# burn-research/OpenMEASURE

Hardware: AMD Instinct MI355X
Metric: SPR fit+reconstruct throughput (GB/s snapshot matrix) (higher is better)
Workload: dtype f64

## Files before the change

### include/spr_hip.h

```cpp
#ifndef SPR_HIP_H
#define SPR_HIP_H

#include <stddef.h>
#include <stdint.h>

#ifdef __cplusplus
extern "C" {
#endif

#define SPR_OK 0
#define SPR_E_INVALID (-1)
#define SPR_E_UNSUPPORTED (-2)
#define SPR_E_HIP (-3)
#define SPR_E_WORKSPACE (-4)

#define SPR_MAX_M 256
#define SPR_MAX_M_WIDE 512
#define SPR_MAX_R 128
#define SPR_MAX_R_STREAM 256
#define SPR_MAX_R_WIDE 1024

#define SPR_ABI_VERSION 5
int spr_abi_version(void);
const char *spr_last_error(void);
int spr_device_cus(int *out_cus);
int spr_upload_bytes(void *d_dst, const void *h_pinned_src, int64_t n_bytes, void *stream);
int spr_download_bytes(void *h_pinned_dst, const void *d_src, int64_t n_bytes, void *h_pinned_ticket, uint64_t ticket_value,
                       void *stream);
int spr_host_tridiag_vectors(const double *h_d, const double *h_e, int32_t m, const double *h_lam, int32_t r, double *h_Z,
                             int32_t iterations);
int spr_host_eig_top(const double *h_G, int32_t m, int32_t r, double *h_lam, double *h_V, void *fn_dsytrd, void *fn_dsterf,
                     void *fn_dormtr);
int spr_host_svd_top(const double *h_M, int32_t m, int32_t r, double *h_S, double *h_V, void *fn_dgebrd, void *fn_dbdsdc,
                     void *fn_dormbr);

size_t spr_stats_gram_workspace(int32_t m, int32_t n_features);
int spr_stats_gram_f64(const double *d_X, int64_t n_rows, int32_t m, int64_t ldx,
                       int64_t row0, int64_t n_points, int32_t n_features, int32_t center,
                       double *d_rowmean, void *d_workspace, size_t workspace_bytes, void *stream);
int spr_stats_gram_finalize_f64(int64_t n_rows, int32_t m, int64_t row0, int64_t n_points,
                                int32_t n_features, const void *d_workspace, size_t workspace_bytes,
                                double *d_fstats, double *d_gram, int32_t ldg, int32_t origin,
                                void *stream);
size_t spr_rowstats_workspace(int32_t n_features);
int spr_rowstats_f64(const double *d_X, int64_t n_rows, int32_t m, int64_t ldx, int64_t row0,
                     int64_t n_points, int32_t n_features, double *d_rowmean, double *d_fstats,
                     void *d_workspace, size_t workspace_bytes, void *stream);
size_t spr_gram_cross_workspace(int32_t m, int32_t n_features);
int spr_gram_cross_f64(const double *d_X, int64_t n_rows, int32_t m, int64_t ldx, int64_t row0,
                       int64_t n_points, int32_t n_features, int32_t center, double *d_rowmean,
                       double *d_gram, void *d_workspace, size_t workspace_bytes, void *stream);
int spr_rowmean_stats_f64(const double *d_rowmean, int64_t n_rows, int64_t row0, int64_t n_points,
                          int32_t n_features, double *d_fstats, void *d_workspace, size_t workspace_bytes,
                          void *stream);
int spr_gram_cross_pair_f64(const double *d_X, int64_t n_rows, int32_t col_a, int32_t col_b, int32_t w_b,
                            int32_t ldg, int64_t ldx, int64_t row0, int64_t n_points, int32_t n_features,
                            int32_t center, double *d_rowmean, double *d_gram, void *d_workspace,
                            size_t workspace_bytes, void *stream);

int32_t spr_spectrum_max_m(void);
int spr_spectrum_f64(const double *d_gram, const double *d_fstats_all, int32_t n_ranks,
                     int32_t n_features, int32_t m, int32_t scale_code, int32_t r, double *d_feat,
                     double *d_scale, double *d_inv_scale, double *d_lam, double *d_S, double *d_expvar,
                     double *d_V, double *d_W, double *d_Ar, double *d_info, void *stream);

int spr_gram_combine_f64(const double *d_gram, const double *d_fstats_all, int32_t n_ranks,
// ... 403 lines not shown
```

### openmeasure_amd/_lib.py

```python
from __future__ import annotations

import ctypes as C
import os

_HERE = os.path.dirname(os.path.abspath(__file__))
LIB_PATH = os.environ.get('SPR_HIP_LIBRARY') or os.path.join(_HERE, 'libspr_hip.so')

SPR_ABI_VERSION = 5
SPR_MAX_M = 256
SPR_MAX_M_WIDE = 512
SPR_MAX_R = 128
SPR_MAX_R_STREAM = 256
SPR_MAX_R_WIDE = 1024
SPR_GP_MAX_M = 800
SPR_GP_MAX_D = 8

_i32, _i64, _u64, _sz = C.c_int32, C.c_int64, C.c_uint64, C.c_size_t
_p = C.c_void_p
_dbl = C.c_double

PROTOTYPES = {
    'spr_abi_version': (C.c_int, []),
    'spr_last_error': (C.c_char_p, []),
    'spr_device_cus': (C.c_int, [C.POINTER(C.c_int)]),
    'spr_upload_bytes': (C.c_int, [_p, _p, _i64, _p]),
    'spr_download_bytes': (C.c_int, [_p, _p, _i64, _p, _u64, _p]),
    'spr_host_tridiag_vectors': (C.c_int, [_p, _p, _i32, _p, _i32, _p, _i32]),
    'spr_host_eig_top': (C.c_int, [_p, _i32, _i32, _p, _p, _p, _p, _p]),
    'spr_host_svd_top': (C.c_int, [_p, _i32, _i32, _p, _p, _p, _p, _p]),
    'spr_stats_gram_workspace': (_sz, [_i32, _i32]),
    'spr_stats_gram_f64': (C.c_int, [_p, _i64, _i32, _i64, _i64, _i64, _i32, _i32, _p, _p, _sz, _p]),
    'spr_stats_gram_finalize_f64': (C.c_int, [_i64, _i32, _i64, _i64, _i32, _p, _sz, _p, _p, _i32, _i32, _p]),
    'spr_stats_gram_shifted_f64': (C.c_int, [_p, _i64, _i32, _i64, _i64, _i64, _i32, _p, _p, _p, _sz, _p]),
    'spr_gram_shift_finish_f64': (C.c_int, [_p, _p, _i64, _i32, _i32, _p, _i32, _p]),
    'spr_rowstats_workspace': (_sz, [_i32]),
    'spr_rowstats_f64': (C.c_int, [_p, _i64, _i32, _i64, _i64, _i64, _i32, _p, _p, _p, _sz, _p]),
    'spr_gram_cross_workspace': (_sz, [_i32, _i32]),
    'spr_gram_cross_f64': (C.c_int, [_p, _i64, _i32, _i64, _i64, _i64, _i32, _i32, _p, _p, _p, _sz, _p]),
    'spr_gram_cross_pair_f64': (C.c_int, [_p, _i64, _i32, _i32, _i32, _i32, _i64, _i64, _i64, _i32, _i32, _p, _p, _p, _sz, _p]),
    'spr_rowmean_stats_f64': (C.c_int, [_p, _i64, _i64, _i64, _i32, _p, _p, _sz, _p]),
    'spr_spectrum_max_m': (_i32, []),
    'spr_spectrum_f64': (C.c_int, [_p, _p, _i32, _i32, _i32, _i32, _i32, _p, _p, _p, _p, _p, _p, _p, _p, _p, _p, _p]),
    'spr_gram_combine_f64': (C.c_int, [_p, _p, _i32, _i32, _i32, _i32, _p, _p, _p, _p, _p]),
    'spr_project_f64': (C.c_int, [_p, _i64, _i32, _i64, _i64, _i64, _i32, _i32, _p, _p, _p, _i32, _p, _i64, _i32, _p]),
    'spr_project_norms_supported': (_i32, [_i32, _i32, _i64, _i64, _p, _i32]),
    'spr_project_norms_f64': (C.c_int, [_p, _i64, _i32, _i64, _i64, _i64, _i32, _i32, _p, _p, _p, _i32, _p, _i64, _p, _p]),
    'spr_project_stream_norms_f64': (C.c_int, [_p, _i64, _i32, _i64, _i64, _i64, _i32, _i32, _p, _p, _p, _i32, _p, _i64, _p, _p, _sz, _p]),
    'spr_project_stream_workspace': (_sz, [_i32, _i32, _i32]),
    'spr_project_stream_f64': (C.c_int, [_p, _i64, _i32, _i64, _i64, _i64, _i32, _i32, _p, _p, _p, _i32, _p, _i64, _p, _sz, _p]),
    'spr_scale_rows_f64': (C.c_int, [_p, _i64, _i32, _i64, _i64, _i64, _i32, _p, _p, _p, _i64, _p]),
    'spr_unscale_f64': (C.c_int, [_p, _i64, _i64, _i64, _i32, _p, _p, _p, _p, _p]),
    'spr_feature_minmax_workspace': (_sz, [_i32]),
    'spr_feature_minmax_f64': (C.c_int, [_p, _i64, _i32, _i64, _i64, _i64, _i32, _p, _p, _sz, _p]),
    'spr_feature_digit_hist_f64': (C.c_int, [_p, _i64, _i32, _i64, _i64, _i64, _i32, _p, _i32, _i32, _i32, _p, _p]),
    'spr_colsums_workspace': (_sz, [_i32, _i32]),
# ... 152 lines not shown
```

### openmeasure_amd/csrc/project_ws.hip

```cpp
#include <type_traits>

#include "rowtile.hpp"
#include "launch.hpp"

namespace {

#ifndef WS_ABLATE
#define WS_ABLATE 0
#endif
constexpr int WS_WAVES = 8;
constexpr int WS_ROWS = 16 * WS_WAVES;

template <int RT> struct WsLds { static constexpr int NC = 16 * RT, LDW = NC; static_assert(RT % 2 == 0, "column tiles come in pairs"); };

template <typename TX> struct WsPiece;
template <> struct WsPiece<double> { f64x2 a, b; };
template <> struct WsPiece<float> { float x, y, z, w; };

template <int VEC, typename TX>
__device__ inline WsPiece<TX> ws_load(const TX *__restrict__ rp, int col0, int m) {
  WsPiece<TX> p;
  if constexpr (std::is_same<TX, double>::value) {
    if (VEC) {
      p.a = *reinterpret_cast<const f64x2 *>(rp + col0);
      p.b = *reinterpret_cast<const f64x2 *>(rp + col0 + 2);
    } else {
      p.a.x = rp[col0 < m ? col0 : 0];         p.a.y = rp[col0 + 1 < m ? col0 + 1 : 0];
      p.b.x = rp[col0 + 2 < m ? col0 + 2 : 0]; p.b.y = rp[col0 + 3 < m ? col0 + 3 : 0];
    }
  } else {
    if (VEC) {
      const float4 v = *reinterpret_cast<const float4 *>(rp + col0);
      p.x = v.x; p.y = v.y; p.z = v.z; p.w = v.w;
    } else {
      p.x = rp[col0 < m ? col0 : 0];         p.y = rp[col0 + 1 < m ? col0 + 1 : 0];
      p.z = rp[col0 + 2 < m ? col0 + 2 : 0]; p.w = rp[col0 + 3 < m ? col0 + 3 : 0];
    }
  }
  return p;
}

template <typename TX>
__device__ inline double ws_elem(const WsPiece<TX> &p, int t) {
  if constexpr (std::is_same<TX, double>::value) return t == 0 ? p.a.x : t == 1 ? p.a.y : t == 2 ? p.b.x : p.b.y;
  else return (double)(t == 0 ? p.x : t == 1 ? p.y : t == 2 ? p.z : p.w);
}

template <int MT, int RT, int VEC, typename TX, typename TU, bool NRM>
__global__ __launch_bounds__(WS_WAVES * 64) void project_ws_kernel(
    const TX *__restrict__ X, int64_t ldx, int m, int center_i, SegPlan plan, const double *__restrict__ inv_scale,
    const double *__restrict__ rowmean, const double *__restrict__ W, int r, TU *__restrict__ Ur, int64_t ldu,
    double *__restrict__ nrm2) {
  constexpr int K = 16 * MT, NJ = MT;
  constexpr int NC = WsLds<RT>::NC, LDW = WsLds<RT>::LDW;
  __shared__ double Wl[K * LDW];

  int f, wl, wpf, base;
  int64_t lo, hi;
  if (!seg_locate(plan, blockIdx.x, f, wl, wpf, base, lo, hi)) return;

  const int lane = threadIdx.x & 63;
  const int wave = __builtin_amdgcn_readfirstlane(threadIdx.x >> 6);
  const int li = lane & 15, kk = lane >> 4;
  const double isc = inv_scale[f];

  for (int e = threadIdx.x; e < K * NC; e += WS_WAVES * 64) {
    const int k = e / NC, c = e - k * NC;
    Wl[k * LDW + (c >> 5) * 32 + (c & 15) * 2 + ((c >> 4) & 1)] = (k < m && c < r) ? W[(int64_t)k * r + c] * isc : 0.0;
  }
  __syncthreads();
  double wbar[RT];
#pragma unroll
  for (int ct = 0; ct < RT; ++ct) {
    double sacc = 0.0;
    if (center_i != 0) {
      for (int k = kk; k < K; k += 4) sacc += Wl[k * LDW + (ct >> 1) * 32 + li * 2 + (ct & 1)];
      sacc += __shfl_xor(sacc, 16, 64);
      sacc += __shfl_xor(sacc, 32, 64);
    }
    wbar[ct] = sacc;
  }

  const int64_t nchunks = (hi - lo + WS_ROWS - 1) / WS_ROWS;
  int64_t c = wl;
  if (c >= nchunks) return;
  const double *wb = Wl + (4 * kk) * LDW + 2 * li;
  const double *wb_hi = wb + 128 * LDW;

  auto row_ptr = [&](int64_t cc) {
    int64_t row = lo + cc * WS_ROWS + 16 * wave + li;
    row = row < hi ? row : hi - 1;
    return X + row * ldx;
  };
  WsPiece<TX> areg[NJ];
  {
    const TX *rp = row_ptr(c);
#pragma unroll
    for (int j = 0; j < NJ; ++j) areg[j] = ws_load<VEC, TX>(rp, 16 * j + 4 * kk, m);
  }
  while (c < nchunks) {
    const int64_t cn = c + wpf;
    const TX *rpn = row_ptr(cn < nchunks ? cn : c);
    const int64_t blk0 = lo + c * WS_ROWS + 16 * wave;
    double mu[4];
#pragma unroll
    for (int i = 0; i < 4; ++i) {
      const int64_t rr = blk0 + kk + 4 * i;
      const double v = rowmean[rr < hi ? rr : hi - 1];
// ... 43 lines not shown
        if (NRM) {
#pragma unroll
          for (int i = 0; i < 4; ++i) { const double v = (double)(TU)s[i]; q[i] = fma(v, v, q[i]); }
        }
        if (full) {
#pragma unroll
          for (int i = 0; i < 4; ++i) up[4 * i * ldu + 16 * ct] = (TU)s[i];
        } else if (16 * ct + li < r) {
#pragma unroll
          for (int i = 0; i < 4; ++i)
            if (blk0 + kk + 4 * i < hi) up[4 * i * ldu + 16 * ct] = (TU)s[i];
        }
      }
      if (NRM) {
#pragma unroll
        for (int i = 0; i < 4; ++i) {
          const double t = group_sum_t<16>(q[i]);
          if (li == i && blk0 + kk + 4 * i < hi) nrm2[blk0 + kk + 4 * i] = t;
        }
      }
    }
    c = cn;
  }
}

template <int MT, int RT, typename TX, typename TU>
int ws_launch(const TX *X, int64_t n_rows, int32_t m, int64_t ldx, int64_t row0, int64_t n_points, int32_t n_features,
              int center, const double *inv_scale, const double *rowmean, const double *W, int32_t r, TU *Ur,
              int64_t ldu, int accumulate, double *nrm2, hipStream_t st) {
  SegPlan plan = spr_make_plan(row0, n_rows, n_points, n_features, WS_ROWS);
  static const int narrow_per_cu = [] { const char *e = getenv("SPR_WS_WG_PER_CU"); const int v = e ? atoi(e) : 2; return v >= 1 && v <= 4 ? v : 2; }();
  const int grid = spr_plan_grid(plan, MT <= 4 ? narrow_per_cu : 1);
  const bool vec = (m == 16 * MT) && spr_rows_aligned16(X, sizeof(TX) * ldx);
  if (!vec) return SPR_E_UNSUPPORTED;
  if (nrm2)
    hipLaunchKernelGGL((project_ws_kernel<MT, RT, 1, TX, TU, true>), dim3(grid), dim3(WS_WAVES * 64), 0, st, X, ldx, (int)m,
                       center, plan, inv_scale, rowmean, W, (int)r, Ur, ldu, nrm2);
  else
    hipLaunchKernelGGL((project_ws_kernel<MT, RT, 1, TX, TU, false>), dim3(grid), dim3(WS_WAVES * 64), 0, st, X, ldx, (int)m,
                       center, plan, inv_scale, rowmean, W, (int)r, Ur, ldu, nrm2);
  SPR_LAUNCH_CHECK();
  return SPR_OK;
}

}

#include "project_ws.hpp"

template <typename TX, typename TU>
int spr_project_ws(const TX *d_X, int64_t n_rows, int32_t m, int64_t ldx, int64_t row0, int64_t n_points,
                   int32_t n_features, int32_t center, const double *d_inv_scale, const double *d_rowmean,
                   const double *d_W, int32_t r, TU *d_Ur, int64_t ldu, int32_t accumulate, double *d_rownorm2,
                   hipStream_t st) {
  if (accumulate) return SPR_E_UNSUPPORTED;
  const int mt = spr_round_mt(m);
  const int need = (r + 15) / 16;
  const int rt = need <= 2 ? 2 : need <= 4 ? 4 : 0;
#define WS(MTV, RTV)                                                                                             \
  if (mt == MTV && rt == RTV)                                                                                    \
    return ws_launch<MTV, RTV, TX, TU>(d_X, n_rows, m, ldx, row0, n_points, n_features, center, d_inv_scale,   \
                                        d_rowmean, d_W, r, d_Ur, ldu, accumulate, d_rownorm2, st)
#ifdef PROJ_WS_LAB
  WS(16, 4);
// ... 19 lines not shown
```

### openmeasure_amd/csrc/stats_gram.hip

```cpp
#include <stdlib.h>

#include <type_traits>

#include "rowtile.hpp"
#include "launch.hpp"

#ifndef GRAM_UNIT_PAIRING
#define GRAM_UNIT_PAIRING 1
#endif
#ifndef GRAM_ABLATE
#define GRAM_ABLATE 0
#endif
#if GRAM_ABLATE == 1
#define GRAM_MFMA(a, b, c) ({ asm volatile("" ::"v"(a), "v"(b)); (c); })
#else
#define GRAM_MFMA(a, b, c) __builtin_amdgcn_mfma_f64_16x16x4f64((a), (b), (c), 0, 0, 0)
#endif

namespace {

template <int MT>
struct GramShape {
  static constexpr int MPAD = 16 * MT;
  static constexpr int MP = MPAD + ((MT % 2 == 0) ? 16 : 0);
  static constexpr int T = MT * (MT + 1) / 2;
  static constexpr int NU = (MT + 1) / 2;
};

// ... 11 lines not shown
template <> struct GramCfg<12> { static constexpr int NW = 12, R = 24, KS = 2; static constexpr bool DBUF = false; static constexpr int LPRMAX = 32; };
#ifndef GRAM_DBUF16
#define GRAM_DBUF16 false
#endif
template <> struct GramCfg<16> { static constexpr int NW = 8,  R = 32, KS = 1; static constexpr bool DBUF = GRAM_DBUF16; static constexpr int LPRMAX = 16; };

template <int MT> struct GramOut { static constexpr int KSO = (GramCfg<MT>::KS >= 4) ? 1 : GramCfg<MT>::KS; };

constexpr int tri_index(int mt, int ti, int tj) { return ti * mt - ti * (ti - 1) / 2 + (tj - ti); }

template <int MT>
__device__ inline void tile_coords(int idx, int &ti, int &tj) {
  ti = 0;
  while (ti < MT - 1 && idx >= MT - ti) { idx -= MT - ti; ++ti; }
  tj = ti + idx;
  if (tj > MT - 1) tj = MT - 1;
}

template <int MT, int U, int VEC, typename TX>
__device__ inline void gram_wave(const TX *__restrict__ X, int64_t ldx, int m, int center,
                                 int64_t lo, int64_t hi, int wl, int wpf, int ks, int wave, int lane,
                                 double *__restrict__ lds0, double *__restrict__ lds1,
                                 double *__restrict__ rowmean, double *__restrict__ stat_part,
                                 double *__restrict__ slab, double *__restrict__ rowsum) {
  using S = GramShape<MT>;
  using C = GramCfg<MT>;
  constexpr int R = C::R, KS = C::KS, NW = C::NW, MP = S::MP, T = S::T;
  constexpr int KROWS = R / KS, KSTEPS = KROWS / 4;
  constexpr int RA = U, RB = MT - 1 - U;
  constexpr int NA = MT - RA;
  constexpr int NB = (RB != RA) ? MT - RB : 0;
  static_assert(KROWS % 4 == 0, "k slice must be a multiple of the MFMA depth");
  using RT = RowTile<MT, R, MP, NW, C::LPRMAX, TX>;

  f64x4 accA[NA];
  f64x4 accB[NB > 0 ? NB : 1];
#pragma unroll
  for (int j = 0; j < NA; ++j) accA[j] = (f64x4){0.0, 0.0, 0.0, 0.0};
#pragma unroll
  for (int j = 0; j < NB; ++j) accB[j] = (f64x4){0.0, 0.0, 0.0, 0.0};

  RowStats st;
  st.init();
  RT tile;

  const int64_t nchunks = (hi - lo + R - 1) / R;
  int64_t c = wl;
// ... 77 lines not shown
        }
#pragma unroll
        for (int j = 0; j < NB; ++j) {
          double *tp = red + tri_index(MT, RB, RB + j) * 256;
          tp[0] = accB[j].x; tp[64] = accB[j].y; tp[128] = accB[j].z; tp[192] = accB[j].w;
        }
      }
      __syncthreads();
      if (ks == s - 1) {
#pragma unroll
        for (int j = 0; j < NA; ++j) {
          const double *tp = red + tri_index(MT, RA, RA + j) * 256;
          accA[j].x += tp[0]; accA[j].y += tp[64]; accA[j].z += tp[128]; accA[j].w += tp[192];
        }
#pragma unroll
        for (int j = 0; j < NB; ++j) {
          const double *tp = red + tri_index(MT, RB, RB + j) * 256;
          accB[j].x += tp[0]; accB[j].y += tp[64]; accB[j].z += tp[128]; accB[j].w += tp[192];
        }
      }
    }
  }
  if (KSO == KS || ks == 0) {
    double *sp = slab + ((int64_t)blockIdx.x * KSO + (KSO == KS ? ks : 0)) * T * 256 + lane;
#pragma unroll
    for (int j = 0; j < NA; ++j) {
      double *tp = sp + (int64_t)tri_index(MT, RA, RA + j) * 256;
      tp[0] = accA[j].x; tp[64] = accA[j].y; tp[128] = accA[j].z; tp[192] = accA[j].w;
    }
#pragma unroll
    for (int j = 0; j < NB; ++j) {
      double *tp = sp + (int64_t)tri_index(MT, RB, RB + j) * 256;
      tp[0] = accB[j].x; tp[64] = accB[j].y; tp[128] = accB[j].z; tp[192] = accB[j].w;
    }
  }
  if ((lane % RT::LPR) == 0) {
    double *q = stat_part + ((int64_t)blockIdx.x * RT::ROWS_PER_IT + wave * RT::RPW + lane / RT::LPR) * 3;
    q[0] = st.cnt; q[1] = st.mean(); q[2] = st.m2();
  }
}

__device__ inline void chan_merge(double &n, double &mu, double &m2, double nb, double mb, double sb) {
  if (nb > 0.0) {
    const double tot = n + nb, d = mb - mu;
    mu += d * nb / tot;
    m2 += sb + d * d * n * nb / tot;
    n = tot;
  }
}

template <int MT, int U, typename TX, bool EXT, bool SUMS>
__device__ inline void gram_wave_own(const TX *__restrict__ X, int64_t ldx, int64_t lo, int64_t hi, int wl, int wpf, int ks,
                                     int wave, int lane, double *__restrict__ lds0, double *__restrict__ lds1,
                                     double *__restrict__ rowmean, double *__restrict__ slab, double *__restrict__ rowsum) {
  using S = GramShape<MT>;
  using C = GramCfg<MT>;
  constexpr int R = C::R, KS = C::KS, NW = C::NW, MP = S::MP, T = S::T;
  constexpr int KROWS = R / KS, KSTEPS = KROWS / 4;
  constexpr int RA = U, RB = MT - 1 - U;
  constexpr int NA = MT - RA;
  constexpr int NB = (RB != RA) ? MT - RB : 0;
  using RT = RowTile<MT, R, MP, NW, C::LPRMAX, TX>;

  f64x4 accA[NA];
  f64x4 accB[NB > 0 ? NB : 1];
#pragma unroll
  for (int j = 0; j < NA; ++j) accA[j] = (f64x4){0.0, 0.0, 0.0, 0.0};
#pragma unroll
  for (int j = 0; j < NB; ++j) accB[j] = (f64x4){0.0, 0.0, 0.0, 0.0};

  RT tile;
  const int64_t nchunks = (hi - lo + R - 1) / R;
  const int64_t lane_off = (int64_t)(wave * RT::RPW + lane / RT::LPR) * ldx;
  auto base_of = [&](int64_t row0) { return X + row0 * ldx; };
  int64_t c = wl;
  int64_t crow0 = lo + c * R;
#pragma unroll
// ... 43 lines not shown
        for (int j = 0; j < NA; ++j) accA[j] = GRAM_MFMA(op[k & 1][0], op[k & 1][j], accA[j]);
#pragma unroll
        for (int j = 0; j < NB; ++j) accB[j] = GRAM_MFMA(op[k & 1][RB - RA], op[k & 1][RB - RA + j], accB[j]);
        if (nfull) stage(std::true_type{}, k); else stage(std::false_type{}, k);
      }
    } else {
#pragma unroll
      for (int k = 0; k < KSTEPS; ++k) {
        double op[NA];
#pragma unroll
        for (int j = 0; j < NA; ++j) op[j] = p[k * 4 * MP + 16 * j];
#pragma unroll
        for (int j = 0; j < NA; ++j) accA[j] = GRAM_MFMA(op[0], op[j], accA[j]);
#pragma unroll
        for (int j = 0; j < NB; ++j) accB[j] = GRAM_MFMA(op[RB - RA], op[RB - RA + j], accB[j]);
        if (nfull) stage(std::true_type{}, k); else stage(std::false_type{}, k);
      }
    }
    buf ^= 1;
    c = cn;
    cn = c2;
    nrow0 = n2row0;
  }
  double *sp = slab + ((int64_t)blockIdx.x * KS + ks) * T * 256 + lane;
#pragma unroll
  for (int j = 0; j < NA; ++j) {
    double *tp = sp + (int64_t)tri_index(MT, RA, RA + j) * 256;
    tp[0] = accA[j].x; tp[64] = accA[j].y; tp[128] = accA[j].z; tp[192] = accA[j].w;
  }
#pragma unroll
  for (int j = 0; j < NB; ++j) {
    double *tp = sp + (int64_t)tri_index(MT, RB, RB + j) * 256;
    tp[0] = accB[j].x; tp[64] = accB[j].y; tp[128] = accB[j].z; tp[192] = accB[j].w;
  }
}

template <int MT, typename TX, bool EXT, bool SUMS>
__global__ __launch_bounds__(GramCfg<MT>::NW * 64) void stats_gram_own_kernel(
    const TX *__restrict__ X, int64_t ldx, SegPlan plan, double *__restrict__ rowmean, double *__restrict__ slab,
    double *__restrict__ rowsum) {
  using S = GramShape<MT>;
  using C = GramCfg<MT>;
  constexpr int NU = S::NU;
  __shared__ double lds[2][C::R * S::MP];
  int f, wl, wpf, base;
  int64_t lo, hi;
  if (!seg_locate(plan, blockIdx.x, f, wl, wpf, base, lo, hi)) return;
  const int lane = threadIdx.x & 63;
  const int wave = __builtin_amdgcn_readfirstlane(threadIdx.x >> 6);
  const int ks = wave / NU;
  const int unit = (GRAM_UNIT_PAIRING && NU == 8 && C::KS == 1) ? ((wave < 4) ? wave : 11 - wave) : wave % NU;
#define GRAM_UNIT(UV)                                                                                          \
  case UV:                                                                                                     \
    if constexpr (UV < NU)                                                                                     \
      gram_wave_own<MT, UV, TX, EXT, SUMS>(X, ldx, lo, hi, wl, wpf, ks, wave, lane, lds[0], lds[1], rowmean, slab, rowsum); \
    break;
  switch (unit) {
    GRAM_UNIT(0) GRAM_UNIT(1) GRAM_UNIT(2) GRAM_UNIT(3) GRAM_UNIT(4) GRAM_UNIT(5) GRAM_UNIT(6) GRAM_UNIT(7)
    default: break;
  }
#undef GRAM_UNIT
}

constexpr int RS_THREADS = 1024;
__global__ __launch_bounds__(RS_THREADS) void gram_rowmean_stats_kernel(const double *__restrict__ rowmean, SegPlan plan,
                                                                        int slots_per_wg, double *__restrict__ stat_part) {
  __shared__ double sn[RS_THREADS / 64], smu[RS_THREADS / 64], sm2[RS_THREADS / 64];
  int f, wl, wpf, base;
  int64_t lo, hi;
  if (!seg_locate(plan, blockIdx.x, f, wl, wpf, base, lo, hi)) return;
  const int lane = threadIdx.x & 63, wave = threadIdx.x >> 6;
  RowStats st;
  st.init();
  const int64_t step = (int64_t)wpf * RS_THREADS;
  int64_t row = lo + (int64_t)wl * RS_THREADS + threadIdx.x;
  for (; row + 3 * step < hi; row += 4 * step) {
    const double a = rowmean[row], b = rowmean[row + step], c = rowmean[row + 2 * step], d = rowmean[row + 3 * step];
    st.push(a, true); st.push(b, true); st.push(c, true); st.push(d, true);
  }
  for (; row < hi; row += step) st.push(rowmean[row], true);
  double n = st.cnt, mu = st.mean(), m2 = st.m2();
  for (int o = 32; o > 0; o >>= 1) {
    const double on = __shfl_down(n, o, 64), om = __shfl_down(mu, o, 64), os = __shfl_down(m2, o, 64);
    chan_merge(n, mu, m2, on, om, os);
  }
  if (lane == 0) { sn[wave] = n; smu[wave] = mu; sm2[wave] = m2; }
  __syncthreads();
  double *q = stat_part + (int64_t)blockIdx.x * slots_per_wg * 3;
  if (threadIdx.x == 0) {
    n = 0.0; mu = 0.0; m2 = 0.0;
    for (int w = 0; w < RS_THREADS / 64; ++w) chan_merge(n, mu, m2, sn[w], smu[w], sm2[w]);
    q[0] = n; q[1] = mu; q[2] = m2;
  }
  for (int e = 3 + threadIdx.x; e < slots_per_wg * 3; e += RS_THREADS) q[e] = 0.0;
}

template <int MT, int VEC, typename TX>
__global__ __launch_bounds__(GramCfg<MT>::NW * 64) void stats_gram_kernel(
    const TX *__restrict__ X, int64_t ldx, int m, int center_i, SegPlan plan,
    double *__restrict__ rowmean, double *__restrict__ stat_part, double *__restrict__ slab, double *__restrict__ rowsum) {
  using S = GramShape<MT>;
  using C = GramCfg<MT>;
  constexpr int NU = S::NU;
  static_assert(NU * C::KS == C::NW, "waves = units x k slices");
  __shared__ double lds[2][C::R * S::MP];

  int f, wl, wpf, base;
  int64_t lo, hi;
  if (!seg_locate(plan, blockIdx.x, f, wl, wpf, base, lo, hi)) return;

  const int lane = threadIdx.x & 63;
  const int wave = __builtin_amdgcn_readfirstlane(threadIdx.x >> 6);
  const int unit = wave % NU, ks = wave / NU;
#define GRAM_UNIT(UV)                                                                                        \
  case UV:                                                                                                   \
    if constexpr (UV < NU)                                                                                   \
      gram_wave<MT, UV, VEC, TX>(X, ldx, m, center_i, lo, hi, wl, wpf, ks, wave, lane, lds[0],    \
                        lds[1], rowmean, stat_part, slab, rowsum);                                           \
    break;
  switch (unit) {
    GRAM_UNIT(0) GRAM_UNIT(1) GRAM_UNIT(2) GRAM_UNIT(3) GRAM_UNIT(4) GRAM_UNIT(5) GRAM_UNIT(6) GRAM_UNIT(7)
    default: break;
  }
#undef GRAM_UNIT
}

template <int MT>
__global__ __launch_bounds__(1024) void gram_finalize_kernel(
    const double *__restrict__ slab, const double *__restrict__ stat_part, int m, SegPlan plan,
    int slots_per_wg, double *__restrict__ gram, double *__restrict__ fstats, int ldg, int origin) {
  constexpr int T = GramShape<MT>::T;
  constexpr int KS = GramOut<MT>::KSO;
  __shared__ double red[4][256];
  const int f = blockIdx.y;
  const int tile = blockIdx.x;
  int base = 0, wpf = 0;
  {
    int acc = 0;
    const int f0 = seg_first_feature(plan), f1 = seg_last_feature(plan);
    for (int ff = f0; ff <= f1; ++ff) {
      int64_t lo, hi;
      seg_range(plan, ff, lo, hi);
      const int w = seg_wgs(plan, hi - lo);
      if (ff == f) { base = acc; wpf = w; }
      acc += w;
    }
  }
  int ti, tj;
  tile_coords<MT>(tile, ti, tj);
  const int e = threadIdx.x & 255, g = threadIdx.x >> 8;
  const int np = wpf * KS;
  const double *sp = slab + ((int64_t)base * KS * T + tile) * 256 + e;
  const int64_t stride = (int64_t)T * 256;
  double s0 = 0.0, s1 = 0.0, s2 = 0.0, s3 = 0.0;
  int p = g;
  for (; p + 12 < np; p += 16) {
    s0 += sp[p * stride];
    s1 += sp[(p + 4) * stride];
    s2 += sp[(p + 8) * stride];
    s3 += sp[(p + 12) * stride];
  }
  for (; p < np; p += 4) s0 += sp[p * stride];
  red[g][e] = (s0 + s1) + (s2 + s3);
  __syncthreads();
  if (g == 0) {
    const double sum = (red[0][e] + red[1][e]) + (red[2][e] + red[3][e]);
    const int l = e & 63, reg = e >> 6;
    const int gi = ti * 16 + (l >> 4) + 4 * reg, gj = tj * 16 + (l & 15);
    if (gi < m && gj < m) {
      double *G = gram + (int64_t)f * ldg * ldg + (int64_t)origin * ldg + origin;
      G[(int64_t)gi * ldg + gj] = sum;
      if (ti != tj) G[(int64_t)gj * ldg + gi] = sum;
    }
  }
  if (tile == 0) {
// ... 21 lines not shown
template <int MT>
int occupancy_wgs() {
  static int cached = 0;
  if (cached) return cached;
  int per_cu = 0;
  if (hipOccupancyMaxActiveBlocksPerMultiprocessor(&per_cu, stats_gram_kernel<MT, 2, double>, GramCfg<MT>::NW * 64, 0) != hipSuccess ||
      per_cu < 1)
    per_cu = 1;
  if (per_cu > 4) per_cu = 4;
  cached = per_cu * spr_cus_or_default();
  return cached;
}

template <int MT>
SegPlan make_plan(int64_t n_rows, int64_t row0, int64_t n_points, int32_t n_features) {
  SegPlan p;
  p.row0 = row0; p.n_rows = n_rows; p.n_points = n_points; p.n_features = n_features;
  p.total_wg = occupancy_wgs<MT>();
  p.chunk_rows = GramCfg<MT>::R;
  return p;
}

template <int MT>
size_t workspace_bytes(int32_t n_features) {
  using RT = RowTile<MT, GramCfg<MT>::R, GramShape<MT>::MP, GramCfg<MT>::NW, GramCfg<MT>::LPRMAX>;
  const int64_t max_grid = (int64_t)occupancy_wgs<MT>() + n_features;
  return (size_t)max_grid * GramCfg<MT>::KS * GramShape<MT>::T * 256 * sizeof(double) +
         (size_t)max_grid * RT::ROWS_PER_IT * 3 * sizeof(double);
}

template <int MT, typename TX>
int launch(const TX *X, int64_t n_rows, int32_t m, int64_t ldx, int64_t row0, int64_t n_points,
           int32_t n_features, int center, double *rowmean, void *ws, size_t ws_bytes, hipStream_t st,
           double *rowsum = nullptr) {
  SPR_REQUIRE(ws_bytes >= workspace_bytes<MT>(n_features), SPR_E_WORKSPACE,
              "spr_stats_gram_f64: workspace %zu < %zu", ws_bytes, workspace_bytes<MT>(n_features));
  SPR_REQUIRE(!rowsum || center == 2, SPR_E_INVALID, "spr_stats_gram: row sums are an output of centre mode 2 only");
  SegPlan plan = make_plan<MT>(n_rows, row0, n_points, n_features);
  const int grid = seg_total_wgs(plan);
  const int64_t max_grid = (int64_t)occupancy_wgs<MT>() + n_features;
  SPR_REQUIRE(grid >= 1 && grid <= max_grid, SPR_E_INVALID, "spr_stats_gram_f64: bad grid %d", grid);
  double *slab = static_cast<double *>(ws);
  double *stat_part = slab + (size_t)max_grid * GramCfg<MT>::KS * GramShape<MT>::T * 256;
  const int lm = spr_load_mode(spr_pair_aligned(X, m, ldx), m, MT);
#define SG_LAUNCH(LM)                                                                                         \
  hipLaunchKernelGGL((stats_gram_kernel<MT, LM, TX>), dim3(grid), dim3(GramCfg<MT>::NW * 64), 0, st, X, ldx, (int)m, \
                     center, plan, rowmean, stat_part, slab, rowsum)
  using RTL = RowTile<MT, GramCfg<MT>::R, GramShape<MT>::MP, GramCfg<MT>::NW, GramCfg<MT>::LPRMAX, TX>;
  static const bool own_on = [] { const char *e = getenv("SPR_GRAM_OWN"); return !(e && e[0] == '0'); }();
  if (MT >= 8 && lm == 2 && (center == 1 || center == 2) && own_on && spr_rows_aligned16(X, sizeof(TX) * ldx)) {
    if constexpr (MT >= 8) {
      if (center == 1)
        hipLaunchKernelGGL((stats_gram_own_kernel<MT, TX, false, false>), dim3(grid), dim3(GramCfg<MT>::NW * 64), 0, st, X, ldx,
                           plan, rowmean, slab, rowsum);
      else if (!rowsum)
        hipLaunchKernelGGL((stats_gram_own_kernel<MT, TX, true, false>), dim3(grid), dim3(GramCfg<MT>::NW * 64), 0, st, X, ldx,
                           plan, rowmean, slab, rowsum);
      else
        hipLaunchKernelGGL((stats_gram_own_kernel<MT, TX, true, true>), dim3(grid), dim3(GramCfg<MT>::NW * 64), 0, st, X, ldx,
                           plan, rowmean, slab, rowsum);
      SPR_LAUNCH_CHECK();
      hipLaunchKernelGGL(gram_rowmean_stats_kernel, dim3(grid), dim3(RS_THREADS), 0, st, rowmean, plan, (int)RTL::ROWS_PER_IT,
                         stat_part);
      SPR_LAUNCH_CHECK();
      return SPR_OK;
    }
  }
  if (lm == 2) SG_LAUNCH(2);
  else if (lm == 1) SG_LAUNCH(1);
  else SG_LAUNCH(0);
#undef SG_LAUNCH
  SPR_LAUNCH_CHECK();
  return SPR_OK;
}

template <int MT>
int launch_finalize(int64_t n_rows, int32_t m, int64_t row0, int64_t n_points, int32_t n_features,
                    double *fstats, double *gram, int ldg, int origin, const void *ws, size_t ws_bytes,
                    hipStream_t st) {
  using RT = RowTile<MT, GramCfg<MT>::R, GramShape<MT>::MP, GramCfg<MT>::NW, GramCfg<MT>::LPRMAX>;
  SPR_REQUIRE(ws_bytes >= workspace_bytes<MT>(n_features), SPR_E_WORKSPACE,
              "spr_stats_gram_finalize_f64: workspace %zu < %zu", ws_bytes, workspace_bytes<MT>(n_features));
  SegPlan plan = make_plan<MT>(n_rows, row0, n_points, n_features);
  const int64_t max_grid = (int64_t)occupancy_wgs<MT>() + n_features;
  const double *slab = static_cast<const double *>(ws);
  const double *stat_part = slab + (size_t)max_grid * GramCfg<MT>::KS * GramShape<MT>::T * 256;
  hipLaunchKernelGGL(gram_finalize_kernel<MT>, dim3(GramShape<MT>::T, n_features), dim3(1024), 0, st, slab,
                     stat_part, (int)m, plan, (int)RT::ROWS_PER_IT, gram, fstats, ldg, origin);
  SPR_LAUNCH_CHECK();
  return SPR_OK;
}

int check_args(const char *who, const void *X, int64_t n_rows, int32_t m, int64_t ldx, int64_t row0,
               int64_t n_points, int32_t n_features) {
  SPR_REQUIRE(X != nullptr, SPR_E_INVALID, "%s: X is NULL", who);
  SPR_REQUIRE(n_rows > 0 && m > 0 && ldx >= m, SPR_E_INVALID, "%s: bad shape n_rows=%lld m=%d ldx=%lld", who,
              (long long)n_rows, m, (long long)ldx);
  SPR_REQUIRE(n_points > 0 && n_features > 0 && row0 >= 0, SPR_E_INVALID, "%s: bad feature layout", who);
  SPR_REQUIRE(row0 + n_rows <= n_points * (int64_t)n_features, SPR_E_INVALID,
              "%s: rows [%lld,%lld) exceed n_points*n_features=%lld", who, (long long)row0,
              (long long)(row0 + n_rows), (long long)(n_points * (int64_t)n_features));
  SPR_REQUIRE(m <= SPR_MAX_M, SPR_E_UNSUPPORTED, "%s: m=%d > %d not built", who, m, SPR_MAX_M);
  return SPR_OK;
}

}

#define GRAM_DISPATCH_M(mt, CALL)            \
  switch (mt) {                              \
    case 1: CALL(1); break;                  \
    case 2: CALL(2); break;                  \
// ... 96 lines not shown
```

Measured before the change: 1170.

## Split rows evenly across workgroups with feature-straddling pieces for gram and projection

Adds an even-split plan that divides the total row chunks across exactly the occupancy-sized grid, so a workgroup may process up to two pieces that cross a feature boundary. The stats/gram and workspace projection kernels loop over these pieces, the gram finalize reads each feature's partial slabs through the new piece table, and row stats run as a separate kernel over the old segment grid. The aim is to remove load imbalance and tail workgroups left by per-feature segment rounding. In exchange it adds extra syncs and weight reloads at piece boundaries and more indexing logic, and it applies only where the plan qualifies.

```diff
diff --git a/include/spr_hip.h b/include/spr_hip.h
--- a/include/spr_hip.h
+++ b/include/spr_hip.h
@@ -42,6 +42,9 @@
                                 int32_t n_features, const void *d_workspace, size_t workspace_bytes,
                                 double *d_fstats, double *d_gram, int32_t ldg, int32_t origin,
                                 void *stream);
+int spr_even_plan_pieces(int64_t row0, int64_t n_rows, int64_t n_points, int32_t n_features, int32_t n_workgroups,
+                         int32_t chunk_rows, int32_t capacity, int64_t *first_row, int64_t *piece_rows, int32_t *feature,
+                         int32_t *owner, int32_t *n_pieces, int32_t *applicable);
 size_t spr_rowstats_workspace(int32_t n_features);
 int spr_rowstats_f64(const double *d_X, int64_t n_rows, int32_t m, int64_t ldx, int64_t row0,
                      int64_t n_points, int32_t n_features, double *d_rowmean, double *d_fstats,
diff --git a/openmeasure_amd/_lib.py b/openmeasure_amd/_lib.py
--- a/openmeasure_amd/_lib.py
+++ b/openmeasure_amd/_lib.py
@@ -31,6 +31,7 @@
     'spr_stats_gram_workspace': (_sz, [_i32, _i32]),
     'spr_stats_gram_f64': (C.c_int, [_p, _i64, _i32, _i64, _i64, _i64, _i32, _i32, _p, _p, _sz, _p]),
     'spr_stats_gram_finalize_f64': (C.c_int, [_i64, _i32, _i64, _i64, _i32, _p, _sz, _p, _p, _i32, _i32, _p]),
+    'spr_even_plan_pieces': (C.c_int, [_i64, _i64, _i64, _i32, _i32, _i32, _i32, _p, _p, _p, _p, _p, _p]),
     'spr_stats_gram_shifted_f64': (C.c_int, [_p, _i64, _i32, _i64, _i64, _i64, _i32, _p, _p, _p, _sz, _p]),
     'spr_gram_shift_finish_f64': (C.c_int, [_p, _p, _i64, _i32, _i32, _p, _i32, _p]),
     'spr_rowstats_workspace': (_sz, [_i32]),
diff --git a/openmeasure_amd/csrc/even_plan.hip b/openmeasure_amd/csrc/even_plan.hip
--- /dev/null
+++ b/openmeasure_amd/csrc/even_plan.hip
@@ -0,0 +1,41 @@
+#include "even_plan.hpp"
+#include "launch.hpp"
+
+extern "C" int spr_even_plan_pieces(int64_t row0, int64_t n_rows, int64_t n_points, int32_t n_features, int32_t n_workgroups,
+                                    int32_t chunk_rows, int32_t capacity, int64_t *first_row, int64_t *piece_rows,
+                                    int32_t *feature, int32_t *owner, int32_t *n_pieces, int32_t *applicable) {
+  SPR_REQUIRE(n_pieces && applicable, SPR_E_INVALID, "spr_even_plan_pieces: NULL output");
+  SPR_REQUIRE(n_rows > 0 && n_workgroups > 0 && chunk_rows > 0, SPR_E_INVALID,
+              "spr_even_plan_pieces: n_rows=%lld n_workgroups=%d chunk_rows=%d", (long long)n_rows, n_workgroups, chunk_rows);
+  SPR_REQUIRE_LAYOUT("spr_even_plan_pieces", row0, n_rows, n_points, n_features);
+  SegPlan plan = spr_make_plan(row0, n_rows, n_points, n_features, chunk_rows);
+  plan.total_wg = n_workgroups;
+  *n_pieces = 0;
+  *applicable = even_plan_applies(plan) ? 1 : 0;
+  if (!*applicable) return SPR_OK;
+  SPR_REQUIRE(capacity == 0 || (first_row && piece_rows && feature && owner), SPR_E_INVALID,
+              "spr_even_plan_pieces: NULL table");
+  int n = 0;
+  for (int b = 0; b < n_workgroups; ++b) {
+    EvenPiece pc[2];
+    const int k = even_locate(plan, b, pc[0], pc[1]);
+    for (int i = 0; i < k; ++i, ++n) {
+      SPR_REQUIRE(n < capacity, SPR_E_WORKSPACE, "spr_even_plan_pieces: more than %d pieces", capacity);
+      SPR_REQUIRE(pc[i].idx == n, SPR_E_INVALID, "spr_even_plan_pieces: piece %d of workgroup %d is numbered %d", n, b, pc[i].idx);
+      first_row[n] = pc[i].lo;
+      piece_rows[n] = pc[i].hi - pc[i].lo;
+      feature[n] = pc[i].f;
+      owner[n] = b;
+    }
+  }
+  for (int f = 0; f < n_features; ++f) {
+    int first, count, t_first = 0, t_count = 0;
+    even_feature_pieces(plan, f, first, count);
+    for (int i = 0; i < n; ++i)
+      if (feature[i] == f && t_count++ == 0) t_first = i;
+    SPR_REQUIRE(count == t_count && (count == 0 || first == t_first), SPR_E_INVALID,
+                "spr_even_plan_pieces: feature %d has pieces [%d,+%d), the table says [%d,+%d)", f, first, count, t_first, t_count);
+  }
+  *n_pieces = n;
+  return SPR_OK;
+}
diff --git a/openmeasure_amd/csrc/even_plan.hpp b/openmeasure_amd/csrc/even_plan.hpp
--- /dev/null
+++ b/openmeasure_amd/csrc/even_plan.hpp
@@ -0,0 +1,98 @@
+#pragma once
+#include <stdlib.h>
+
+#include "common.hpp"
+
+struct EvenPiece {
+  int64_t lo, hi;
+  int32_t f;
+  int32_t idx;
+};
+
+__host__ __device__ inline int64_t even_seg_chunks(const SegPlan &p, int f) {
+  int64_t lo, hi;
+  seg_range(p, f, lo, hi);
+  return (hi - lo + p.chunk_rows - 1) / p.chunk_rows;
+}
+
+__host__ __device__ inline int64_t even_total_chunks(const SegPlan &p) {
+  int64_t tot = 0;
+  const int f1 = seg_last_feature(p);
+  for (int f = seg_first_feature(p); f <= f1; ++f) tot += even_seg_chunks(p, f);
+  return tot;
+}
+
+__host__ __device__ inline int64_t even_wg_begin(int64_t C, int G, int64_t b) { return C * b / G; }
+__host__ __device__ inline int64_t even_wg_of_chunk(int64_t C, int G, int64_t q) { return ((q + 1) * G - 1) / C; }
+
+__host__ __device__ inline int even_locate(const SegPlan &p, int b, EvenPiece &p0, EvenPiece &p1) {
+  const int G = p.total_wg;
+  const int64_t C = even_total_chunks(p);
+  if (b < 0 || b >= G) return 0;
+  const int64_t s = even_wg_begin(C, G, b), e = even_wg_begin(C, G, (int64_t)b + 1);
+  if (s >= e) return 0;
+  const int64_t R = p.chunk_rows;
+  const int f0 = seg_first_feature(p), f1 = seg_last_feature(p);
+  int64_t acc = 0, idx = b;
+  for (int f = f0; f <= f1; ++f) {
+    if (f > f0 && acc < s && even_wg_begin(C, G, even_wg_of_chunk(C, G, acc)) != acc) ++idx;
+    const int64_t n = even_seg_chunks(p, f);
+    if (s < acc + n) {
+      int64_t lo, hi;
+      seg_range(p, f, lo, hi);
+      const int64_t e0 = e < acc + n ? e : acc + n;
+      p0.f = f;
+      p0.idx = (int32_t)idx;
+      p0.lo = lo + (s - acc) * R;
+      p0.hi = lo + (e0 - acc) * R < hi ? lo + (e0 - acc) * R : hi;
+      if (e <= acc + n || f == f1) return 1;
+      seg_range(p, f + 1, lo, hi);
+      p1.f = f + 1;
+      p1.idx = (int32_t)idx + 1;
+      p1.lo = lo;
+      p1.hi = lo + (e - acc - n) * R < hi ? lo + (e - acc - n) * R : hi;
+      return 2;
+    }
+    acc += n;
+  }
+  return 0;
+}
+
+__host__ __device__ inline void even_feature_pieces(const SegPlan &p, int f, int &first, int &count) {
+  first = 0;
+  count = 0;
+  const int f0 = seg_first_feature(p), f1 = seg_last_feature(p);
+  if (f < f0 || f > f1) return;
+  const int G = p.total_wg;
+  const int64_t C = even_total_chunks(p);
+  int64_t acc = 0, inside = 0;
+  for (int ff = f0; ff <= f; ++ff) {
+    if (ff > f0 && even_wg_begin(C, G, even_wg_of_chunk(C, G, acc)) != acc) ++inside;
+    if (ff < f) acc += even_seg_chunks(p, ff);
+  }
+  const int64_t n = even_seg_chunks(p, f);
+  const int64_t w0 = even_wg_of_chunk(C, G, acc), w1 = even_wg_of_chunk(C, G, acc + n - 1);
+  first = (int)(w0 + inside);
+  count = (int)(w1 - w0 + 1);
+}
+
+inline bool even_plan_applies(const SegPlan &p) {
+  const int G = p.total_wg;
+  if (G < 1 || p.chunk_rows < 1 || p.n_rows < 1) return false;
+  const int64_t C = even_total_chunks(p);
+  if (C < G) return false;
+  const int f0 = seg_first_feature(p), f1 = seg_last_feature(p);
+  int64_t acc = even_seg_chunks(p, f0);
+  for (int f = f0 + 1; f < f1; ++f) {
+    const int64_t n = even_seg_chunks(p, f);
+    const int64_t b = even_wg_of_chunk(C, G, acc - 1);
+    if (even_wg_begin(C, G, b + 1) > acc + n) return false;
+    acc += n;
+  }
+  return true;
+}
+
+inline bool spr_even_split_on() {
+  static const bool on = [] { const char *e = getenv("SPR_EVEN_SPLIT"); return !(e && e[0] == '0'); }();
+  return on;
+}
diff --git a/openmeasure_amd/csrc/project_ws.hip b/openmeasure_amd/csrc/project_ws.hip
--- a/openmeasure_amd/csrc/project_ws.hip
+++ b/openmeasure_amd/csrc/project_ws.hip
@@ -2,6 +2,7 @@
 
 #include "rowtile.hpp"
 #include "launch.hpp"
+#include "even_plan.hpp"
 
 namespace {
 
@@ -48,22 +49,30 @@
 
 template <int MT, int RT, int VEC, typename TX, typename TU, bool NRM>
 __global__ __launch_bounds__(WS_WAVES * 64) void project_ws_kernel(
-    const TX *__restrict__ X, int64_t ldx, int m, int center_i, SegPlan plan, const double *__restrict__ inv_scale,
+    const TX *__restrict__ X, int64_t ldx, int m, int center_i, SegPlan plan, int even, const double *__restrict__ inv_scale,
     const double *__restrict__ rowmean, const double *__restrict__ W, int r, TU *__restrict__ Ur, int64_t ldu,
     double *__restrict__ nrm2) {
   constexpr int K = 16 * MT, NJ = MT;
   constexpr int NC = WsLds<RT>::NC, LDW = WsLds<RT>::LDW;
   __shared__ double Wl[K * LDW];
 
-  int f, wl, wpf, base;
-  int64_t lo, hi;
-  if (!seg_locate(plan, blockIdx.x, f, wl, wpf, base, lo, hi)) return;
+  int wl = 0, wpf = 1, npieces = 1;
+  EvenPiece pc0 = {0, 0, 0, 0}, pc1 = pc0;
+  if (MT >= 8 && even) {
+    npieces = even_locate(plan, blockIdx.x, pc0, pc1);
+  } else {
+    int base;
+    if (!seg_locate(plan, blockIdx.x, pc0.f, wl, wpf, base, pc0.lo, pc0.hi)) return;
+  }
 
   const int lane = threadIdx.x & 63;
   const int wave = __builtin_amdgcn_readfirstlane(threadIdx.x >> 6);
   const int li = lane & 15, kk = lane >> 4;
-  const double isc = inv_scale[f];
-
+  for (int pc = 0; pc < (MT >= 8 ? npieces : 1); ++pc) {
+  const int64_t lo = pc ? pc1.lo : pc0.lo, hi = pc ? pc1.hi : pc0.hi;
+  const double isc = inv_scale[pc ? pc1.f : pc0.f];
+
+  if (pc) __syncthreads();
   for (int e = threadIdx.x; e < K * NC; e += WS_WAVES * 64) {
     const int k = e / NC, c = e - k * NC;
     Wl[k * LDW + (c >> 5) * 32 + (c & 15) * 2 + ((c >> 4) & 1)] = (k < m && c < r) ? W[(int64_t)k * r + c] * isc : 0.0;
@@ -83,7 +92,7 @@
 
   const int64_t nchunks = (hi - lo + WS_ROWS - 1) / WS_ROWS;
   int64_t c = wl;
-  if (c >= nchunks) return;
+  if (c >= nchunks) continue;
   const double *wb = Wl + (4 * kk) * LDW + 2 * li;
   const double *wb_hi = wb + 128 * LDW;
 
@@ -173,6 +182,7 @@
     }
     c = cn;
   }
+  }
 }
 
 template <int MT, int RT, typename TX, typename TU>
@@ -181,15 +191,17 @@
               int64_t ldu, int accumulate, double *nrm2, hipStream_t st) {
   SegPlan plan = spr_make_plan(row0, n_rows, n_points, n_features, WS_ROWS);
   static const int narrow_per_cu = [] { const char *e = getenv("SPR_WS_WG_PER_CU"); const int v = e ? atoi(e) : 2; return v >= 1 && v <= 4 ? v : 2; }();
-  const int grid = spr_plan_grid(plan, MT <= 4 ? narrow_per_cu : 1);
+  int grid = spr_plan_grid(plan, MT <= 4 ? narrow_per_cu : 1);
+  const int even = (MT >= 8 && spr_even_split_on() && even_plan_applies(plan)) ? 1 : 0;
+  if (even) grid = plan.total_wg;
   const bool vec = (m == 16 * MT) && spr_rows_aligned16(X, sizeof(TX) * ldx);
   if (!vec) return SPR_E_UNSUPPORTED;
   if (nrm2)
     hipLaunchKernelGGL((project_ws_kernel<MT, RT, 1, TX, TU, true>), dim3(grid), dim3(WS_WAVES * 64), 0, st, X, ldx, (int)m,
-                       center, plan, inv_scale, rowmean, W, (int)r, Ur, ldu, nrm2);
+                       center, plan, even, inv_scale, rowmean, W, (int)r, Ur, ldu, nrm2);
   else
     hipLaunchKernelGGL((project_ws_kernel<MT, RT, 1, TX, TU, false>), dim3(grid), dim3(WS_WAVES * 64), 0, st, X, ldx, (int)m,
-                       center, plan, inv_scale, rowmean, W, (int)r, Ur, ldu, nrm2);
+                       center, plan, even, inv_scale, rowmean, W, (int)r, Ur, ldu, nrm2);
   SPR_LAUNCH_CHECK();
   return SPR_OK;
 }
diff --git a/openmeasure_amd/csrc/stats_gram.hip b/openmeasure_amd/csrc/stats_gram.hip
--- a/openmeasure_amd/csrc/stats_gram.hip
+++ b/openmeasure_amd/csrc/stats_gram.hip
@@ -4,6 +4,7 @@
 
 #include "rowtile.hpp"
 #include "launch.hpp"
+#include "even_plan.hpp"
 
 #ifndef GRAM_UNIT_PAIRING
 #define GRAM_UNIT_PAIRING 1
@@ -61,7 +62,7 @@
                                  int64_t lo, int64_t hi, int wl, int wpf, int ks, int wave, int lane,
                                  double *__restrict__ lds0, double *__restrict__ lds1,
                                  double *__restrict__ rowmean, double *__restrict__ stat_part,
-                                 double *__restrict__ slab, double *__restrict__ rowsum) {
+                                 double *__restrict__ slab, double *__restrict__ rowsum, int slab_idx, bool write_stats) {
   using S = GramShape<MT>;
   using C = GramCfg<MT>;
   constexpr int R = C::R, KS = C::KS, NW = C::NW, MP = S::MP, T = S::T;
@@ -185,7 +186,7 @@
     }
   }
   if (KSO == KS || ks == 0) {
-    double *sp = slab + ((int64_t)blockIdx.x * KSO + (KSO == KS ? ks : 0)) * T * 256 + lane;
+    double *sp = slab + ((int64_t)slab_idx * KSO + (KSO == KS ? ks : 0)) * T * 256 + lane;
 #pragma unroll
     for (int j = 0; j < NA; ++j) {
       double *tp = sp + (int64_t)tri_index(MT, RA, RA + j) * 256;
@@ -197,7 +198,7 @@
       tp[0] = accB[j].x; tp[64] = accB[j].y; tp[128] = accB[j].z; tp[192] = accB[j].w;
     }
   }
-  if ((lane % RT::LPR) == 0) {
+  if (write_stats && (lane % RT::LPR) == 0) {
     double *q = stat_part + ((int64_t)blockIdx.x * RT::ROWS_PER_IT + wave * RT::RPW + lane / RT::LPR) * 3;
     q[0] = st.cnt; q[1] = st.mean(); q[2] = st.m2();
   }
@@ -215,7 +216,8 @@
 template <int MT, int U, typename TX, bool EXT, bool SUMS>
 __device__ inline void gram_wave_own(const TX *__restrict__ X, int64_t ldx, int64_t lo, int64_t hi, int wl, int wpf, int ks,
                                      int wave, int lane, double *__restrict__ lds0, double *__restrict__ lds1,
-                                     double *__restrict__ rowmean, double *__restrict__ slab, double *__restrict__ rowsum) {
+                                     double *__restrict__ rowmean, double *__restrict__ slab, double *__restrict__ rowsum,
+                                     int slab_idx) {
   using S = GramShape<MT>;
   using C = GramCfg<MT>;
   constexpr int R = C::R, KS = C::KS, NW = C::NW, MP = S::MP, T = S::T;
@@ -305,7 +307,7 @@
     cn = c2;
     nrow0 = n2row0;
   }
-  double *sp = slab + ((int64_t)blockIdx.x * KS + ks) * T * 256 + lane;
+  double *sp = slab + ((int64_t)slab_idx * KS + ks) * T * 256 + lane;
 #pragma unroll
   for (int j = 0; j < NA; ++j) {
     double *tp = sp + (int64_t)tri_index(MT, RA, RA + j) * 256;
@@ -318,17 +320,30 @@
   }
 }
 
+constexpr int GRAM_EVEN_MIN_MT = 16;
+#define GRAM_LOCATE_PIECES                                                                       \
+  int wl = 0, wpf = 1, npieces = 1;                                                              \
+  EvenPiece pc0 = {0, 0, 0, (int32_t)blockIdx.x}, pc1 = pc0;                                     \
+  if (MT >= GRAM_EVEN_MIN_MT && even) {  \
+    npieces = even_locate(plan, blockIdx.x, pc0, pc1);                                           \
+  } else {                                                                                       \
+    int f_, base_;                                                                               \
+    if (!seg_locate(plan, blockIdx.x, f_, wl, wpf, base_, pc0.lo, pc0.hi)) return;               \
+  }
+#define GRAM_PIECE(pc)                                   \
+  if (pc) __syncthreads();                               \
+  const int64_t lo = pc ? pc1.lo : pc0.lo, hi = pc ? pc1.hi : pc0.hi; \
+  const int slab_idx = pc ? pc1.idx : pc0.idx;
+
 template <int MT, typename TX, bool EXT, bool SUMS>
 __global__ __launch_bounds__(GramCfg<MT>::NW * 64) void stats_gram_own_kernel(
-    const TX *__restrict__ X, int64_t ldx, SegPlan plan, double *__restrict__ rowmean, double *__restrict__ slab,
+    const TX *__restrict__ X, int64_t ldx, SegPlan plan, int even, double *__restrict__ rowmean, double *__restrict__ slab,
     double *__restrict__ rowsum) {
   using S = GramShape<MT>;
   using C = GramCfg<MT>;
   constexpr int NU = S::NU;
   __shared__ double lds[2][C::R * S::MP];
-  int f, wl, wpf, base;
-  int64_t lo, hi;
-  if (!seg_locate(plan, blockIdx.x, f, wl, wpf, base, lo, hi)) return;
+  GRAM_LOCATE_PIECES
   const int lane = threadIdx.x & 63;
   const int wave = __builtin_amdgcn_readfirstlane(threadIdx.x >> 6);
   const int ks = wave / NU;
@@ -336,11 +351,15 @@
 #define GRAM_UNIT(UV)                                                                                          \
   case UV:                                                                                                     \
     if constexpr (UV < NU)                                                                                     \
-      gram_wave_own<MT, UV, TX, EXT, SUMS>(X, ldx, lo, hi, wl, wpf, ks, wave, lane, lds[0], lds[1], rowmean, slab, rowsum); \
+      gram_wave_own<MT, UV, TX, EXT, SUMS>(X, ldx, lo, hi, wl, wpf, ks, wave, lane, lds[0], lds[1], rowmean, slab, rowsum, \
+                                           slab_idx);                                                          \
     break;
-  switch (unit) {
-    GRAM_UNIT(0) GRAM_UNIT(1) GRAM_UNIT(2) GRAM_UNIT(3) GRAM_UNIT(4) GRAM_UNIT(5) GRAM_UNIT(6) GRAM_UNIT(7)
-    default: break;
+  for (int pc = 0; pc < (MT >= GRAM_EVEN_MIN_MT ? npieces : 1); ++pc) {
+    GRAM_PIECE(pc)
+    switch (unit) {
+      GRAM_UNIT(0) GRAM_UNIT(1) GRAM_UNIT(2) GRAM_UNIT(3) GRAM_UNIT(4) GRAM_UNIT(5) GRAM_UNIT(6) GRAM_UNIT(7)
+      default: break;
+    }
   }
 #undef GRAM_UNIT
 }
@@ -380,17 +399,14 @@
 
 template <int MT, int VEC, typename TX>
 __global__ __launch_bounds__(GramCfg<MT>::NW * 64) void stats_gram_kernel(
-    const TX *__restrict__ X, int64_t ldx, int m, int center_i, SegPlan plan,
+    const TX *__restrict__ X, int64_t ldx, int m, int center_i, SegPlan plan, int even,
     double *__restrict__ rowmean, double *__restrict__ stat_part, double *__restrict__ slab, double *__restrict__ rowsum) {
   using S = GramShape<MT>;
   using C = GramCfg<MT>;
   constexpr int NU = S::NU;
   static_assert(NU * C::KS == C::NW, "waves = units x k slices");
   __shared__ double lds[2][C::R * S::MP];
-
-  int f, wl, wpf, base;
-  int64_t lo, hi;
-  if (!seg_locate(plan, blockIdx.x, f, wl, wpf, base, lo, hi)) return;
+  GRAM_LOCATE_PIECES
 
   const int lane = threadIdx.x & 63;
   const int wave = __builtin_amdgcn_readfirstlane(threadIdx.x >> 6);
@@ -399,18 +415,21 @@
   case UV:                                                                                                   \
     if constexpr (UV < NU)                                                                                   \
       gram_wave<MT, UV, VEC, TX>(X, ldx, m, center_i, lo, hi, wl, wpf, ks, wave, lane, lds[0],    \
-                        lds[1], rowmean, stat_part, slab, rowsum);                                           \
+                        lds[1], rowmean, stat_part, slab, rowsum, slab_idx, !even);                          \
     break;
-  switch (unit) {
-    GRAM_UNIT(0) GRAM_UNIT(1) GRAM_UNIT(2) GRAM_UNIT(3) GRAM_UNIT(4) GRAM_UNIT(5) GRAM_UNIT(6) GRAM_UNIT(7)
-    default: break;
+  for (int pc = 0; pc < (MT >= GRAM_EVEN_MIN_MT ? npieces : 1); ++pc) {
+    GRAM_PIECE(pc)
+    switch (unit) {
+      GRAM_UNIT(0) GRAM_UNIT(1) GRAM_UNIT(2) GRAM_UNIT(3) GRAM_UNIT(4) GRAM_UNIT(5) GRAM_UNIT(6) GRAM_UNIT(7)
+      default: break;
+    }
   }
 #undef GRAM_UNIT
 }
 
 template <int MT>
 __global__ __launch_bounds__(1024) void gram_finalize_kernel(
-    const double *__restrict__ slab, const double *__restrict__ stat_part, int m, SegPlan plan,
+    const double *__restrict__ slab, const double *__restrict__ stat_part, int m, SegPlan plan, int even,
     int slots_per_wg, double *__restrict__ gram, double *__restrict__ fstats, int ldg, int origin) {
   constexpr int T = GramShape<MT>::T;
   constexpr int KS = GramOut<MT>::KSO;
@@ -429,11 +448,13 @@
       acc += w;
     }
   }
+  int sbase = base, scount = wpf;
+  if (even) even_feature_pieces(plan, f, sbase, scount);
   int ti, tj;
   tile_coords<MT>(tile, ti, tj);
   const int e = threadIdx.x & 255, g = threadIdx.x >> 8;
-  const int np = wpf * KS;
-  const double *sp = slab + ((int64_t)base * KS * T + tile) * 256 + e;
+  const int np = scount * KS;
+  const double *sp = slab + ((int64_t)sbase * KS * T + tile) * 256 + e;
   const int64_t stride = (int64_t)T * 256;
   double s0 = 0.0, s1 = 0.0, s2 = 0.0, s3 = 0.0;
   int p = g;
@@ -501,6 +522,11 @@
 }
 
 template <int MT>
+bool use_even_plan(const SegPlan &plan) {
+  return MT >= GRAM_EVEN_MIN_MT && spr_even_split_on() && even_plan_applies(plan);
+}
+
+template <int MT>
 size_t workspace_bytes(int32_t n_features) {
   using RT = RowTile<MT, GramCfg<MT>::R, GramShape<MT>::MP, GramCfg<MT>::NW, GramCfg<MT>::LPRMAX>;
   const int64_t max_grid = (int64_t)occupancy_wgs<MT>() + n_features;
@@ -516,30 +542,33 @@
               "spr_stats_gram_f64: workspace %zu < %zu", ws_bytes, workspace_bytes<MT>(n_features));
   SPR_REQUIRE(!rowsum || center == 2, SPR_E_INVALID, "spr_stats_gram: row sums are an output of centre mode 2 only");
   SegPlan plan = make_plan<MT>(n_rows, row0, n_points, n_features);
-  const int grid = seg_total_wgs(plan);
+  const int seg_grid = seg_total_wgs(plan);
+  const int even = use_even_plan<MT>(plan) ? 1 : 0;
+  const int grid = even ? plan.total_wg : seg_grid;
   const int64_t max_grid = (int64_t)occupancy_wgs<MT>() + n_features;
-  SPR_REQUIRE(grid >= 1 && grid <= max_grid, SPR_E_INVALID, "spr_stats_gram_f64: bad grid %d", grid);
+  SPR_REQUIRE(grid >= 1 && grid <= max_grid && seg_grid >= 1 && seg_grid <= max_grid, SPR_E_INVALID,
+              "spr_stats_gram_f64: bad grid %d", grid);
   double *slab = static_cast<double *>(ws);
   double *stat_part = slab + (size_t)max_grid * GramCfg<MT>::KS * GramShape<MT>::T * 256;
   const int lm = spr_load_mode(spr_pair_aligned(X, m, ldx), m, MT);
 #define SG_LAUNCH(LM)                                                                                         \
   hipLaunchKernelGGL((stats_gram_kernel<MT, LM, TX>), dim3(grid), dim3(GramCfg<MT>::NW * 64), 0, st, X, ldx, (int)m, \
-                     center, plan, rowmean, stat_part, slab, rowsum)
+                     center, plan, even, rowmean, stat_part, slab, rowsum)
   using RTL = RowTile<MT, GramCfg<MT>::R, GramShape<MT>::MP, GramCfg<MT>::NW, GramCfg<MT>::LPRMAX, TX>;
   static const bool own_on = [] { const char *e = getenv("SPR_GRAM_OWN"); return !(e && e[0] == '0'); }();
   if (MT >= 8 && lm == 2 && (center == 1 || center == 2) && own_on && spr_rows_aligned16(X, sizeof(TX) * ldx)) {
     if constexpr (MT >= 8) {
       if (center == 1)
         hipLaunchKernelGGL((stats_gram_own_kernel<MT, TX, false, false>), dim3(grid), dim3(GramCfg<MT>::NW * 64), 0, st, X, ldx,
-                           plan, rowmean, slab, rowsum);
+                           plan, even, rowmean, slab, rowsum);
       else if (!rowsum)
         hipLaunchKernelGGL((stats_gram_own_kernel<MT, TX, true, false>), dim3(grid), dim3(GramCfg<MT>::NW * 64), 0, st, X, ldx,
-                           plan, rowmean, slab, rowsum);
+                           plan, even, rowmean, slab, rowsum);
       else
         hipLaunchKernelGGL((stats_gram_own_kernel<MT, TX, true, true>), dim3(grid), dim3(GramCfg<MT>::NW * 64), 0, st, X, ldx,
-                           plan, rowmean, slab, rowsum);
+                           plan, even, rowmean, slab, rowsum);
       SPR_LAUNCH_CHECK();
-      hipLaunchKernelGGL(gram_rowmean_stats_kernel, dim3(grid), dim3(RS_THREADS), 0, st, rowmean, plan, (int)RTL::ROWS_PER_IT,
+      hipLaunchKernelGGL(gram_rowmean_stats_kernel, dim3(seg_grid), dim3(RS_THREADS), 0, st, rowmean, plan, (int)RTL::ROWS_PER_IT,
                          stat_part);
       SPR_LAUNCH_CHECK();
       return SPR_OK;
@@ -550,6 +579,11 @@
   else SG_LAUNCH(0);
 #undef SG_LAUNCH
   SPR_LAUNCH_CHECK();
+  if (even) {
+    hipLaunchKernelGGL(gram_rowmean_stats_kernel, dim3(seg_grid), dim3(RS_THREADS), 0, st, rowmean, plan, (int)RTL::ROWS_PER_IT,
+                       stat_part);
+    SPR_LAUNCH_CHECK();
+  }
   return SPR_OK;
 }
 
@@ -565,7 +599,7 @@
   const double *slab = static_cast<const double *>(ws);
   const double *stat_part = slab + (size_t)max_grid * GramCfg<MT>::KS * GramShape<MT>::T * 256;
   hipLaunchKernelGGL(gram_finalize_kernel<MT>, dim3(GramShape<MT>::T, n_features), dim3(1024), 0, st, slab,
-                     stat_part, (int)m, plan, (int)RT::ROWS_PER_IT, gram, fstats, ldg, origin);
+                     stat_part, (int)m, plan, use_even_plan<MT>(plan) ? 1 : 0, (int)RT::ROWS_PER_IT, gram, fstats, ldg, origin);
   SPR_LAUNCH_CHECK();
   return SPR_OK;
 }
```

Result: no change. 1179 (median of 6 runs) (+0.8%).
